# pzimbrod/fem-glass-tempering

Measured on AMD Instinct MI355X. Metric: DOF-updates/sec (coupled thermo-visco time step, 3D CG1 hex), higher is better.
Workload: dtype f64; 1 GPU; C4 3D plate CG1/CG1 400x400x50 hex (8200851 T-dofs), dt 0.1, coupled 6-term Prony; parallelism=single GPU, one partition (no communication), output=none (reference writes VTX/XDMF every step), krylov_form=PETSc KSPCG, geometric-multigrid V-cycle preconditioner, preconditioner=gmg, visco_fields=state (T, Tf, Tf_partial, phi, xi, s_tilde, sigma_tilde, sigma)

## Files before the change

### fem-glass-tempering_amd/csrc/tv_internal.h

```cpp
#pragma once
#include <hip/hip_runtime.h>
#include <cstdint>
#include <string>
#include <type_traits>
#include <vector>

#include "tvfem.h"

namespace tv {

constexpr int kWave = 64;
constexpr int kSeg = kWave - 2;
constexpr int kBlock = 256;

enum { kMemDoubles = 0, kMemOther = 1 };
template <class T>
constexpr int mem_kind() {
  return std::is_same<T, double>::value ? kMemDoubles : kMemOther;
}
hipError_t tv_dev_alloc(void** p, size_t bytes, int kind);
hipError_t tv_dev_free(void* p);
template <class T>
inline hipError_t tv_dev_alloc(T** p, size_t bytes, int kind) {
  void* q = nullptr;
// ... 263 lines not shown
                       const double* gface, double omega, double* r, double* dx, double* x0, int it_host, int init,
                       hipStream_t s);
int launch_dg_bpost(const DgGrid& g, const PcgState* st, const double* x0, const double* r, const double* w,
                    const double* gface, double omega, double* z, double* partials, const RedTail* tail, hipStream_t s);

void launch_visco(int dim, int all, const ViscoConst& c, const ViscoFields& f, hipStream_t s);
void launch_visco_Tpass(int dim, int all, const ViscoConst& c, const ViscoFields& f, hipStream_t s);
void launch_visco_Spass(int dim, int all, const ViscoConst& c, const ViscoFields& f, hipStream_t s);

struct EnsArgs {
  int n_bars, nb_pad, n_nodes;
  int n_steps;
  int step_base;
  int thermal_only;
  int max_it;
  double rtol, atol;
  double dt, sigma_sb;
  const double* cm;
  const double* ck;
  const double* htc;
  const double* T_amb;
  const double* eps;
  const double* f;
  double* T;
  double* Tp;
  double* scr;
  int* its_last;
  int* failed_step;
  int64_t* newton_total;
};
struct EnsExt {
  int n_stages;
  int n_probes;
  int every, max_records;
  const int* stage_end;
  const double* htc;
  const double* T_amb;
  const double* eps;
  const int* probes;
  double* hist;
};
void launch_ensemble(const EnsArgs& a, const ViscoConst& c, const ViscoFields& f, const EnsExt* x, hipStream_t s);
void launch_ensemble_dg(const EnsArgs& a, const ViscoConst& c, const ViscoFields& f, const EnsExt* x, hipStream_t s);

constexpr int kVecBlocks = 1024;
constexpr int kVecBlocksMin = 256;
constexpr int kVecNodesPerThread = 16;
constexpr int kVecBlocksMax = 8192;
void launch_pcg_init(int64_t n, const double* r, const double* dinv, double* z, double* dx,
                     double* partials, hipStream_t s);
struct FaceAdd {
  int on;
  int n0, n1, n2;
  int64_t t_off;
  double inv_n0, inv_plane;
  const double* ff[6];
};
FaceAdd cg_face_add(const CgGrid& g, int64_t t_off);


struct MgXfer {
  int fn[3], cn[3];
  int coarse[3];
  int f_kb, f_ke, c_kb, c_ke;
  const int* pi[3];
  const double* pw[3];
  const int* ri[3];
  const double* rw[3];
  int aligned;
};
void launch_mg_restrict(const MgXfer& x, const PcgState* st, const double* bf, const double* wf, const FaceAdd* fa,
                        const double* mask, double* bc, const double* dinv_c, double omega_c, double* xc,
                        hipStream_t s);
struct RRAxis {
  const int* f0;
  const double* w;
};
struct RRArgs {
  int on;
  int fn[3], cn[3];
  RRAxis ax[3];
  double da;
  int raxis, nseg, qchunk;
};
constexpr int kRRQMaxChunk = 64;
bool launch_mg_rrestrict(const RRArgs& a, const PcgState* st, const double* b, const double* x, const FaceAdd& fa,
                         double* bc, const double* dinv_c, double omega_c, double* xc, hipStream_t s);
void launch_cg_facet_faces(const CgGrid& g, const double* T, const double* x, const PcgState* st, hipStream_t s);
FaceAdd cg_face_add_all(const CgGrid& g);

struct CoarsePost {
  const double* b;
  const double* w;
  const double* dinv;
  double omega;
  FaceAdd fa;
};
void launch_mg_prolong(const MgXfer& x, const PcgState* st, double* xf, const double* xc, const double* mask,
                       hipStream_t s, const CoarsePost* cp = nullptr);
bool mg_prolong_smooths(const MgXfer& x);
bool mg_restrict_folds_faces(const MgXfer& x);
void launch_mg_jacobi(int64_t n, const PcgState* st, const double* b, const double* w, const FaceAdd* fa,
                      const double* dinv, double omega, double* x, int mode, hipStream_t s);
void launch_mg_inject(const MgXfer& x, const double* Tf, double* Tc, hipStream_t s);
void launch_mg_inject_range(const MgXfer& x, const double* Tf, double* Tc, int k0, int k1, hipStream_t s);
void launch_mg_resid(int64_t n, const PcgState* st, const double* b, double* w, const FaceAdd* fa, const double* mask,
                     hipStream_t s);
void launch_mg_ownmask(int64_t n, int64_t own0, int64_t own1, const double* dinv, double* mask, hipStream_t s);
constexpr int kMgPrepMax = 4;
struct MgPrep {
  int nlev;
  const double* Tbase;
  MgXfer xf[kMgPrepMax];
  double* T[kMgPrepMax];
  double* dinv[kMgPrepMax];
  CgGrid g[kMgPrepMax];
  int64_t off_n[kMgPrepMax + 1];
  int64_t off_b[kMgPrepMax + 1];
};
void launch_mg_prepare(const MgPrep& p, hipStream_t s);
bool cg_uses_march(const CgGrid& g);
void launch_mg_dg_restrict(const DgGrid& g, const PcgState* st, const double* bf, const double* wf, const double* mask,
                           double* bc, const double* dinv_c, double omega_c, double* xc, int kg0, hipStream_t s);
void launch_mg_dg_prolong(const DgGrid& g, const PcgState* st, double* xf, const double* xc, const double* mask,
                          int kg0, hipStream_t s);
void launch_mg_dg_T(const DgGrid& g, const double* Tdg, double* Tcg, int kg0, hipStream_t s);
int launch_mg_pow(int64_t n, const double* dinv, double* y, double* partials, hipStream_t s);
void launch_mg_scale(int64_t n, const double* y, double a, double* x, hipStream_t s);
bool launch_cg_japply_tail(const CgGrid& g, const double* T, const double* x, double* y, const PcgState* st,
                           double* partials, const RedTail* tail, hipStream_t s);
void launch_cg_japply_partial(const CgGrid& g, const double* T, const double* x, double* y, const PcgState* st,
                              hipStream_t s);
void launch_mg_update(int64_t n, const PcgState* st, const double* pA, const double* pB, const double* w,
                      const FaceAdd* fa, const double* dinv, double omega, double* r, double* dx, double* x0,
                      int it_host, int init, hipStream_t s, const double* lag = nullptr,
                      unsigned* counter = nullptr);
void launch_mg_update_cgs(int64_t n, const PcgState* st, const double* u, double* s, const double* z, double* p,
                          double* dx, double* r, const double* dinv, double omega, double* x0, bool first,
                          const double* lag, int lag_kind, unsigned* counter, hipStream_t stream);
int launch_cg_japply_post(const CgGrid& g, const double* T, const double* x, const double* r, const double* dinv,
                          double omega, double* z, const PcgState* st, double* partials, const RedTail* tail,
                          hipStream_t s);
int launch_mg_post(int64_t n, const PcgState* st, const double* x0, const double* r, const double* w,
                   const FaceAdd* fa, const double* dinv, double omega, double* z, double* partials,
                   const RedTail* tail, hipStream_t s);

void launch_pcg_update(int64_t n, PcgState* st, const double* pA, const double* pB, const double* w,
                       const double* dinv, double* dx, double* z, double* partials, hipStream_t s,
                       const RedTail* tail = nullptr, const FaceAdd* fa = nullptr, int it_host = 0);
void launch_pcg_dx_tail(int64_t n, const PcgState* st, const double* pA, const double* pB, double* dx, int its,
                        hipStream_t s);
void launch_mg_dx_finish(int64_t n, const PcgState* st, const double* pA, const double* pB, double* dx, int its,
                         hipStream_t s);
void launch_reduce_logic(const double* partials, int n, int W, double* out, PcgState* st, int kind,
                         int check_done, hipStream_t s);
void launch_logic(PcgState* st, const double* sums, int kind, hipStream_t s);
void launch_set_state(PcgState* st, const PcgState& h, hipStream_t s, const double* gate = nullptr);
void launch_newton_update(int64_t n, double* T, const double* dx, double* partials, hipStream_t s,
                          const RedTail* tail = nullptr);
void launch_post_group(int64_t n, const PcgState* st, const double* pA, const double* pB, double* dx, double* T,
                       double* partials, double* sums, hipStream_t s);
int pcg_vec_blocks(int64_t n);
void launch_fill(double* x, int64_t n, double v, hipStream_t s);

struct Output;
Output* output_create(const std::string& dir, int dim, const std::vector<std::vector<double>>& Xs, const int* phys,
                      std::string& err);
Output* output_create_unstructured(const std::string& dir, int dim, const std::vector<double>& xyz,
// ... 13 lines not shown
```

### fem-glass-tempering_amd/csrc/tv_mg.hip

```cpp
#include <algorithm>
#include <cstdlib>
#include <type_traits>

#include "tv_stencil.h"

namespace tv {
namespace {

template <bool MASK>
__global__ __launch_bounds__(kBlock) void k_mg_restrict(MgXfer x, const PcgState* __restrict__ st,
                                                        const double* __restrict__ bf,
                                                        const double* __restrict__ wf,
                                                        const double* __restrict__ mask, double* __restrict__ bc,
                                                        const double* __restrict__ dinv_c, double omega_c,
                                                        double* __restrict__ xc) {
  if (st != nullptr && st->done) return;
  const int plane = x.cn[0] * x.cn[1];
  const int n = plane * (x.c_ke - x.c_kb);
  const int fpl = x.fn[0] * x.fn[1];
  const int per = (n + (int)gridDim.x - 1) / (int)gridDim.x;
  const int t0 = xcd_remap(blockIdx.x, gridDim.x) * per, t1 = min(n, t0 + per);
  int k = (t0 + (int)threadIdx.x) / plane, j, i;
  {
    const int rem = t0 + (int)threadIdx.x - k * plane;
// ... 528 lines not shown
      if (xc != nullptr) xc[o] = omega_c * dinv_c[o] * acc;
    }
  };
  if (mask != nullptr) run(std::true_type{});
  else run(std::false_type{});
}

__global__ __launch_bounds__(kBlock) void k_mg_dg_prolong(DgGrid g, const PcgState* __restrict__ st,
                                                          double* __restrict__ xf, const double* __restrict__ xc,
                                                          const double* __restrict__ mask, int ck0, int ck1, int kg0) {
  if (st != nullptr && st->done) return;
  const int c0 = g.c0, c1 = g.c1, n0 = c0 + 1, n1 = c1 + 1;
  const int64_t pc = (int64_t)c0 * c1, ncell = pc * (ck1 - ck0);
  auto run = [&](auto masked) {
    constexpr bool MASKED = decltype(masked)::value;
    for (int64_t cell = blockIdx.x * (int64_t)kBlock + threadIdx.x; cell < ncell; cell += (int64_t)gridDim.x * kBlock) {
      const int i = (int)(cell % c0), j = (int)((cell / c0) % c1), k = ck0 + (int)(cell / pc);
      const DgL a = dg_lay(g, k);
      double xv[8], cv[8], mv[8];
#pragma unroll
      for (int l = 0; l < 8; ++l) {
        const int64_t v = (i + (l & 1)) + (int64_t)n0 * ((j + ((l >> 1) & 1)) + (int64_t)n1 * (k + kg0 + (l >> 2)));
        const int64_t f = a.base + (int64_t)l * a.stride + i + (int64_t)c0 * j;
        xv[l] = xf[f];
        cv[l] = xc[v];
        mv[l] = MASKED ? mask[f] : 1.0;
      }
#pragma unroll
      for (int l = 0; l < 8; ++l) {
        const int64_t f = a.base + (int64_t)l * a.stride + i + (int64_t)c0 * j;
        xf[f] = (MASKED && mv[l] == 0.0) ? 0.0 : xv[l] + cv[l];
      }
    }
  };
  if (mask != nullptr) run(std::true_type{});
  else run(std::false_type{});
}

__global__ __launch_bounds__(kBlock) void k_mg_dg_T(DgGrid g, const double* __restrict__ Tdg, double* __restrict__ Tcg,
                                                    int v0, int v1, int kg0) {
  const int c0 = g.c0, c1 = g.c1, c2 = g.c2, n0 = c0 + 1, n1 = c1 + 1;
  const int64_t nv = (int64_t)n0 * n1 * (v1 - v0);
  for (int64_t v = blockIdx.x * (int64_t)kBlock + threadIdx.x; v < nv; v += (int64_t)gridDim.x * kBlock) {
    const int i = (int)(v % n0), j = (int)((v / n0) % n1), K = v0 + (int)(v / ((int64_t)n0 * n1));
    double s = 0.0;
    int cnt = 0;
#pragma unroll
    for (int l = 0; l < 8; ++l) {
      const int ci = i - (l & 1), cj = j - ((l >> 1) & 1), ck = K - (l >> 2);
      if (ci < 0 || ci >= c0 || cj < 0 || cj >= c1 || ck < 0 || ck >= c2) continue;
      const DgL a = dg_lay(g, ck);
      s += Tdg[a.base + (int64_t)l * a.stride + ci + (int64_t)c0 * cj];
      ++cnt;
    }
    Tcg[i + (int64_t)n0 * (j + (int64_t)n1 * (K + kg0))] = s / cnt;
  }
}

__global__ __launch_bounds__(kBlock) void k_mg_pow(int64_t n, const double* __restrict__ dinv, double* __restrict__ y,
                                                   double* __restrict__ partials) {
  __shared__ double red[kBlock / kWave];
  double acc = 0.0;
  for (int64_t t = blockIdx.x * (int64_t)kBlock + threadIdx.x; t < n; t += (int64_t)gridDim.x * kBlock) {
    const double v = dinv ? dinv[t] * y[t] : y[t];
    y[t] = v;
    acc += v * v;
  }
  acc = wave_sum64(acc);
  if ((threadIdx.x & 63) == 0) red[threadIdx.x >> 6] = acc;
  __syncthreads();
  if (threadIdx.x == 0) partials[blockIdx.x] = (red[0] + red[1]) + (red[2] + red[3]);
}

__global__ __launch_bounds__(kBlock) void k_mg_scale(int64_t n, const double* __restrict__ y, double a,
                                                     double* __restrict__ x) {
  for (int64_t t = blockIdx.x * (int64_t)kBlock + threadIdx.x; t < n; t += (int64_t)gridDim.x * kBlock) x[t] = a * y[t];
}

int blocks_for(int64_t n) { return (int)std::max<int64_t>(1, std::min<int64_t>((n + kBlock - 1) / kBlock, 8192)); }
int xfer_blocks(int64_t n) { return (int)std::max<int64_t>(1, (n + kBlock - 1) / kBlock); }

constexpr int kRRSeg = kWave - 2;
constexpr int kRRWaves = 8;
constexpr int kRRRows = 2 * kRRWaves + 3;
constexpr int kRRPer = (kRRRows + kRRWaves - 1) / kRRWaves;
constexpr int kRRQMax = kRRQMaxChunk;
constexpr int kRRPF = 1;

using rr_buf = __amdgpu_buffer_rsrc_t;
__device__ __forceinline__ rr_buf rr_rsrc(const void* p, uint32_t bytes) {
  const uint64_t a = (uint64_t)p;
  const uint32_t lo = __builtin_amdgcn_readfirstlane((uint32_t)a);
  const uint32_t hi = __builtin_amdgcn_readfirstlane((uint32_t)(a >> 32));
  void* q = (void*)(((uint64_t)hi << 32) | lo);
  return __builtin_amdgcn_make_buffer_rsrc(q, (short)0, (int)__builtin_amdgcn_readfirstlane(bytes), 0x00020000);
}
__device__ __forceinline__ d2a8 rr_ld2(rr_buf r, uint32_t voff, uint32_t soff) {
  typedef unsigned int u4 __attribute__((ext_vector_type(4)));
  const u4 v = __builtin_amdgcn_raw_buffer_load_b128(r, (int)voff, (int)soff, 0);
  return __builtin_bit_cast(d2a8, v);
}
__device__ __forceinline__ d2a8 rr_tail(d2a8 v, bool tail) { return tail ? d2a8{v.y, 0.0} : v; }
__device__ __forceinline__ double rr_ld1(rr_buf r, uint32_t voff) {
  return __builtin_bit_cast(double, __builtin_amdgcn_raw_buffer_load_b64(r, (int)voff, 0, 0));
}

struct RRSet {
  d2a8 xv[kRRPer], bv[kRRPer];
  double fx[kRRPer];
  d2a8 fr;
};

template <int RA>
__global__ __launch_bounds__(kRRWaves * kWave) void k_mg_rrestrict(RRArgs a, const PcgState* __restrict__ st,
                                                                   const double* __restrict__ b,
                                                                   const double* __restrict__ x, FaceAdd fa,
                                                                   double* __restrict__ bc,
                                                                   const double* __restrict__ dinv_c, double omega_c,
                                                                   double* __restrict__ xc) {
  if (st != nullptr && st->done) return;
  __shared__ double sq[kRRQMax][15];
  __shared__ double sr[kRRWaves][15];
  __shared__ double red[2][3][kRRRows][kWave];
  const int lane = threadIdx.x & (kWave - 1);
  const int wave = __builtin_amdgcn_readfirstlane((int)threadIdx.x >> 6);
  constexpr int ra = RA, qa = 3 - RA;
  const int ncr = a.cn[ra], ncq = a.cn[qa];
  const int nrb = (ncr + kRRWaves - 1) / kRRWaves;
  const int bid = xcd_remap(blockIdx.x, gridDim.x);
  const int seg = bid % a.nseg;
  const int t = bid / a.nseg;
  const int rb = t % nrb, chunk = t / nrb;
  const int Jc0 = rb * kRRWaves;
  const int Jc = Jc0 + wave;
  const bool row_ok = Jc < ncr;
  const int Jcc = row_ok ? Jc : ncr - 1;
  const int Q0 = chunk * a.qchunk, Q1 = min(Q0 + a.qchunk, ncq);
  const int nf0 = a.fn[0], ncx = a.cn[0];
  const int nfr = a.fn[ra], nfq = a.fn[qa];
  const int I = seg * kRRSeg - 1 + lane;
  const bool Iok = I >= 0 && I < ncx;
  const int e0 = 2 * I;
  {
    const int tid = threadIdx.x;
    for (int e = tid; e < 15 * (Q1 - Q0); e += kRRWaves * kWave) sq[e / 15][e % 15] = a.ax[qa].w[15 * Q0 + e];
    if (lane < 15) sr[wave][lane] = row_ok ? a.ax[ra].w[15 * Jcc + lane] : 0.0;
  }
  const int Jlast = min(Jc0 + kRRWaves, ncr) - 1;
  const int fr_first = kld(a.ax[ra].f0, Jc0);
  const int nrows = kld(a.ax[ra].f0, Jlast) + 5 - fr_first;
  const int my0 = kld(a.ax[ra].f0, Jcc) - fr_first;
  const int sR = (ra == 1) ? nf0 : nf0 * a.fn[1];
  const int sQ = (ra == 1) ? nf0 * a.fn[1] : nf0;
  int frow[kRRPer];
  uint32_t rowoff[kRRPer];
  bool rload[kRRPer];
#pragma unroll
  for (int u = 0; u < kRRPer; ++u) {
    const int sl = wave + u * kRRWaves;
    rload[u] = sl < nrows;
    frow[u] = min(max(fr_first + sl, 0), nfr - 1);
    rowoff[u] = (uint32_t)(sR * frow[u]) * 8u;
  }
  const uint32_t nbytes = (uint32_t)a.fn[0] * (uint32_t)a.fn[1] * (uint32_t)a.fn[2] * 8u;
  const rr_buf rx = rr_rsrc(x, nbytes), rbv = rr_rsrc(b, nbytes);
  const bool xtail = Iok && e0 == nf0 - 1;
  const uint32_t voff = Iok ? (uint32_t)(e0 - (xtail ? 1 : 0)) * 8u : 0x40000000u;
  const bool xl0 = fa.ff[0] != nullptr && e0 == 0, xl1 = fa.ff[1] != nullptr && e0 == nf0 - 1;
  const int n1 = a.fn[1];
  const double* fxb = fa.ff[0] ? fa.ff[0] : fa.ff[1];
  const int64_t dx1 = (fa.ff[0] && fa.ff[1]) ? (int64_t)(fa.ff[1] - fa.ff[0]) : 0;
  const rr_buf rfx = rr_rsrc(fxb, fxb ? (uint32_t)((dx1 + (int64_t)n1 * a.fn[2]) * 8) : 0u);
  const uint32_t fxo = xl1 ? (uint32_t)dx1 : 0u;
  const uint32_t nfa = nbytes / (uint32_t)nfr, nfb = nbytes / (uint32_t)nfq;
  const rr_buf frl = rr_rsrc(fa.ff[2 * ra], fa.ff[2 * ra] ? nfa : 0u);
  const rr_buf frh = rr_rsrc(fa.ff[2 * ra + 1], fa.ff[2 * ra + 1] ? nfa : 0u);
  const rr_buf fql = rr_rsrc(fa.ff[2 * qa], fa.ff[2 * qa] ? nfb : 0u);
  const rr_buf fqh = rr_rsrc(fa.ff[2 * qa + 1], fa.ff[2 * qa + 1] ? nfb : 0u);
  const bool hrl = fa.ff[2 * ra] != nullptr, hrh = fa.ff[2 * ra + 1] != nullptr;
  const bool hql = fa.ff[2 * qa] != nullptr, hqh = fa.ff[2 * qa + 1] != nullptr;
  int uf = -1;
  bool uf_lo = false;
#pragma unroll
  for (int u = 0; u < kRRPer; ++u) {
    const int fr = fr_first + wave + u * kRRWaves;
    if (rload[u] && ((hrl && fr == 0) || (hrh && fr == nfr - 1))) {
      uf = u;
      uf_lo = hrl && fr == 0;
    }
  }
  const rr_buf frs = uf_lo ? frl : frh;
  const int f0q = kld(a.ax[qa].f0, Q0);
  const int np = 2 * (Q1 - Q0) + 3;
  auto fetch = [&](int P, RRSet& S) {
    const int fq = min(max(f0q + P, 0), nfq - 1);
    const uint32_t po = (uint32_t)(sQ * fq) * 8u;
#pragma unroll
    for (int u = 0; u < kRRPer; ++u) {
      S.xv[u] = rr_ld2(rx, rload[u] ? voff : 0x40000000u, rowoff[u] + po);
      S.bv[u] = rr_ld2(rbv, rload[u] ? voff : 0x40000000u, rowoff[u] + po);
    }
#pragma unroll
    for (int u = 0; u < kRRPer; ++u) {
      const int j = (ra == 1) ? frow[u] : fq, k = (ra == 1) ? fq : frow[u];
      S.fx[u] = rr_ld1(rfx, ((xl0 || xl1) && rload[u]) ? (fxo + (uint32_t)(j + n1 * k)) * 8u : 0x40000000u);
    }
    S.fr = rr_ld2(frs, uf >= 0 ? voff : 0x40000000u, (uint32_t)(nf0 * fq) * 8u);
  };
  double wx[15];
#pragma unroll
  for (int m = 0; m < 15; ++m) wx[m] = (Iok ? a.ax[0].w[15 * (Iok ? I : 0) + m] : 0.0);
  auto reduce = [&](int P, const RRSet& S) {
    const int fqr = f0q + P;
    const bool qlo = hql && fqr == 0, qhi = hqh && fqr == nfq - 1;
    d2a8 sv[kRRPer];
#pragma unroll
    for (int u = 0; u < kRRPer; ++u) {
      sv[u] = rr_tail(S.bv[u], xtail);
      sv[u].x -= S.fx[u];
      if (u == uf) {
        const d2a8 f = rr_tail(S.fr, xtail);
        sv[u].x -= f.x;
        sv[u].y -= f.y;
      }
      if (qlo || qhi) {
        const d2a8 f = rr_tail(rr_ld2(qlo ? fql : fqh, voff, (uint32_t)(nf0 * frow[u]) * 8u), xtail);
        sv[u].x -= f.x;
        sv[u].y -= f.y;
      }
    }
    const int buf = P & 1;
#pragma unroll
    for (int u = 0; u < kRRPer; ++u) {
      const d2a8 xv = rr_tail(S.xv[u], xtail);
      const double x0 = shr1(xv.x), x1 = shr1(xv.y), x4 = shl1(xv.x);
      const double s0 = shr1(sv[u].x), s1 = shr1(sv[u].y), s4 = shl1(sv[u].x);
      const double p = ((wx[0] * x0 + wx[1] * x1) + wx[2] * xv.x) + (wx[3] * xv.y + wx[4] * x4);
      const double q = ((wx[5] * x0 + wx[6] * x1) + wx[7] * xv.x) + (wx[8] * xv.y + wx[9] * x4);
      const double s = ((wx[10] * s0 + wx[11] * s1) + wx[12] * sv[u].x) + (wx[13] * sv[u].y + wx[14] * s4);
      const int sl = wave + u * kRRWaves;
      if (sl < kRRRows) {
        red[buf][0][sl][lane] = p;
        red[buf][1][sl][lane] = q;
        red[buf][2][sl][lane] = s;
      }
    }
  };
  auto fold = [&](int P, double& U, double& V, double& Sv) {
    const int buf = P & 1;
    double um = 0.0, uk = 0.0, vv = 0.0, ss = 0.0;
#pragma unroll
    for (int m = 0; m < 5; ++m) {
      const int sl = min(my0 + m, kRRRows - 1);
      const double p = red[buf][0][sl][lane], q = red[buf][1][sl][lane], s = red[buf][2][sl][lane];
      um += sr[wave][m] * (p + a.da * q);
      uk += sr[wave][5 + m] * p;
      vv += sr[wave][m] * p;
      ss += sr[wave][10 + m] * s;
    }
    U = um + a.da * uk;
    V = vv;
    Sv = ss;
  };
  auto contrib = [&](int Q, int m, double U, double V, double Sv) {
    const double* w = sq[Q - Q0];
    return w[10 + m] * Sv - (w[m] * U + a.da * (w[5 + m] * V));
  };
  const bool out_lane = row_ok && Iok && lane >= 1 && lane <= kRRSeg;
  const int nQ = Q1 - Q0;
  double X = 0.0, Y = 0.0;
  const uint32_t ncb = (uint32_t)ncx * (uint32_t)a.cn[1] * (uint32_t)a.cn[2] * 8u;
  const rr_buf rdc = rr_rsrc(dinv_c, xc != nullptr ? ncb : 0u);
  auto coarse_off = [&](int Q) -> uint32_t {
    const int J1 = (ra == 1) ? Jc : Q, K2 = (ra == 1) ? Q : Jc;
    return ((uint32_t)I + (uint32_t)ncx * ((uint32_t)J1 + (uint32_t)a.cn[1] * (uint32_t)K2)) * 8u;
  };
  RRSet S[kRRPF + 1];
#pragma unroll
  for (int s = 0; s < kRRPF; ++s) fetch(min(s, np - 1), S[s]);
  __syncthreads();
#pragma unroll 1
  for (int P0 = 0; P0 < np; P0 += kRRPF + 1) {
#pragma unroll
    for (int s = 0; s <= kRRPF; ++s) {
      const int P = P0 + s;
      const bool completes = P < np && (P & 1) == 0 && (P >> 1) - 2 >= 0 && out_lane;
      const double dcv = rr_ld1(rdc, completes ? coarse_off(Q0 + (P >> 1) - 2) : 0x40000000u);
      __builtin_amdgcn_sched_barrier(0);
      fetch(min(P + kRRPF, np - 1), S[(s + kRRPF) % (kRRPF + 1)]);
      if (P < np) {
        reduce(P, S[s]);
        __syncthreads();
        double U, V, Sv;
        fold(P, U, V, Sv);
        const int k = P >> 1;
        if ((P & 1) == 0) {
          if (k - 2 >= 0 && k - 2 < nQ) X += contrib(Q0 + k - 2, 4, U, V, Sv);
          if (k - 1 >= 0 && k - 1 < nQ) Y += contrib(Q0 + k - 1, 2, U, V, Sv);
          const double Z = (k < nQ) ? contrib(Q0 + k, 0, U, V, Sv) : 0.0;
          if (completes) {
            const int64_t o = coarse_off(Q0 + k - 2) / 8u;
            bc[o] = X;
            if (xc != nullptr) xc[o] = omega_c * dcv * X;
          }
          X = Y;
          Y = Z;
        } else {
          if (k - 1 >= 0 && k - 1 < nQ) X += contrib(Q0 + k - 1, 3, U, V, Sv);
          if (k < nQ) Y += contrib(Q0 + k, 1, U, V, Sv);
        }
      }
    }
  }
}

}



void launch_mg_restrict(const MgXfer& x, const PcgState* st, const double* bf, const double* wf, const FaceAdd* fa,
                        const double* mask, double* bc, const double* dinv_c, double omega_c, double* xc,
                        hipStream_t s) {
  const bool faces = fa != nullptr && fa->on;
  const int64_t n = (int64_t)x.cn[0] * x.cn[1] * (x.c_ke - x.c_kb);
  if (n <= 0) return;
  if (mg_restrict_folds_faces(x)) {
    const int nseg = (x.cn[0] + kPairSeg - 1) / kPairSeg;
    const dim3 g((unsigned)((int64_t)x.cn[1] * (x.c_ke - x.c_kb) * nseg));
    const FaceAdd f = faces ? *fa : FaceAdd{};
#define TV_RP(M, F) \
  hipLaunchKernelGGL((k_mg_restrict_pairs<M, F>), g, dim3(kWave), 0, s, x, st, bf, wf, mask, bc, dinv_c, omega_c, xc, \
                     nseg, f)
    if (mask != nullptr) {
      if (faces) TV_RP(true, true);
      else TV_RP(true, false);
    } else {
      if (faces) TV_RP(false, true);
      else TV_RP(false, false);
    }
#undef TV_RP
    return;
  }
  if (mask != nullptr)
    hipLaunchKernelGGL(k_mg_restrict<true>, dim3(xfer_blocks(n)), dim3(kBlock), 0, s, x, st, bf, wf, mask, bc, dinv_c,
                       omega_c, xc);
  else
    hipLaunchKernelGGL(k_mg_restrict<false>, dim3(xfer_blocks(n)), dim3(kBlock), 0, s, x, st, bf, wf, mask, bc,
                       dinv_c, omega_c, xc);
}

bool mg_restrict_folds_faces(const MgXfer& x) { return x.coarse[0] && x.fn[0] >= 3; }

bool launch_mg_rrestrict(const RRArgs& a, const PcgState* st, const double* b, const double* x, const FaceAdd& fa,
                         double* bc, const double* dinv_c, double omega_c, double* xc, hipStream_t s) {
  const int ncr = a.cn[a.raxis], ncq = a.cn[3 - a.raxis];
  const int nrb = (ncr + kRRWaves - 1) / kRRWaves;
  if (a.qchunk < 1 || a.qchunk > kRRQMax) return false;
  const int nch = (ncq + a.qchunk - 1) / a.qchunk;
  const dim3 g((unsigned)((int64_t)a.nseg * nrb * nch)), bl(kRRWaves * kWave);
  if (a.raxis == 1) hipLaunchKernelGGL(k_mg_rrestrict<1>, g, bl, 0, s, a, st, b, x, fa, bc, dinv_c, omega_c, xc);
  else hipLaunchKernelGGL(k_mg_rrestrict<2>, g, bl, 0, s, a, st, b, x, fa, bc, dinv_c, omega_c, xc);
  return true;
}

bool mg_prolong_blocks(const MgXfer& x) {
  return x.aligned && x.coarse[0] && x.coarse[1] && x.coarse[2] && x.fn[0] >= 3 && x.f_kb == 0;
}

bool mg_prolong_smooths(const MgXfer& x) { return mg_prolong_blocks(x); }

void launch_mg_prolong(const MgXfer& x, const PcgState* st, double* xf, const double* xc, const double* mask,
                       hipStream_t s, const CoarsePost* cp) {
  const int64_t n = (int64_t)x.fn[0] * x.fn[1] * (x.f_ke - x.f_kb);
  if (n <= 0) return;
  if (cp != nullptr && !mg_prolong_smooths(x)) {
    const int64_t nc = (int64_t)x.cn[0] * x.cn[1] * x.cn[2];
    launch_mg_jacobi(nc, st, cp->b, cp->w, &cp->fa, cp->dinv, cp->omega, const_cast<double*>(xc), 1, s);
    cp = nullptr;
  }
  if (mg_prolong_blocks(x)) {
    const int nseg = ((x.fn[0] + 1) / 2 + kPairSeg - 1) / kPairSeg;
    const int nbj = (x.fn[1] + 1) / 2, nbk = (x.f_ke + 1) / 2;
    if (cp != nullptr)
      hipLaunchKernelGGL(k_mg_prolong_blk<true>, dim3((unsigned)((int64_t)nbj * nbk * nseg)), dim3(kWave), 0, s, x, st,
                         xf, xc, mask, nseg, nbj, *cp);
    else
      hipLaunchKernelGGL(k_mg_prolong_blk<false>, dim3((unsigned)((int64_t)nbj * nbk * nseg)), dim3(kWave), 0, s, x, st,
                         xf, xc, mask, nseg, nbj, CoarsePost{});
    return;
  }
  if (x.coarse[0] && x.fn[0] >= 3) {
    const int nseg = ((x.fn[0] + 1) / 2 + kPairSeg - 1) / kPairSeg;
    const int64_t rows = (int64_t)x.fn[1] * (x.f_ke - x.f_kb);
    hipLaunchKernelGGL(k_mg_prolong_pairs, dim3((unsigned)(rows * nseg)), dim3(kWave), 0, s, x, st, xf, xc, mask, nseg);
    return;
  }
  hipLaunchKernelGGL(k_mg_prolong, dim3((unsigned)((n + kPU * kBlock - 1) / (kPU * kBlock))), dim3(kBlock), 0, s, x, st, xf, xc, mask);
}

void launch_mg_jacobi(int64_t n, const PcgState* st, const double* b, const double* w, const FaceAdd* fa,
                      const double* dinv, double omega, double* x, int mode, hipStream_t s) {
  if (n <= 0) return;
  const FaceAdd f = (fa && fa->on) ? *fa : FaceAdd{};
  const dim3 g(blocks_for(n)), bl(kBlock);
  if (mode == 0) hipLaunchKernelGGL((k_mg_jacobi<0, false>), g, bl, 0, s, n, st, b, w, f, dinv, omega, x);
  else if (f.on) hipLaunchKernelGGL((k_mg_jacobi<1, true>), g, bl, 0, s, n, st, b, w, f, dinv, omega, x);
  else hipLaunchKernelGGL((k_mg_jacobi<1, false>), g, bl, 0, s, n, st, b, w, f, dinv, omega, x);
}

void launch_mg_inject(const MgXfer& x, const double* Tf, double* Tc, hipStream_t s) {
  launch_mg_inject_range(x, Tf, Tc, 0, x.cn[2], s);
}

void launch_mg_inject_range(const MgXfer& x, const double* Tf, double* Tc, int k0, int k1, hipStream_t s) {
  const int nxb = (x.cn[0] + kBlock - 1) / kBlock;
  const int64_t rows = (int64_t)x.cn[1] * (k1 - k0);
  if (rows > 0) hipLaunchKernelGGL(k_mg_inject, dim3((unsigned)(rows * nxb)), dim3(kBlock), 0, s, x, Tf, Tc, nxb, k0);
}

void launch_mg_resid(int64_t n, const PcgState* st, const double* b, double* w, const FaceAdd* fa, const double* mask,
                     hipStream_t s) {
  if (n <= 0) return;
  const FaceAdd f = (fa && fa->on) ? *fa : FaceAdd{};
  if (f.on) hipLaunchKernelGGL((k_mg_resid<true>), dim3(blocks_for(n)), dim3(kBlock), 0, s, n, st, b, w, f, mask);
  else hipLaunchKernelGGL((k_mg_resid<false>), dim3(blocks_for(n)), dim3(kBlock), 0, s, n, st, b, w, f, mask);
}

void launch_mg_ownmask(int64_t n, int64_t own0, int64_t own1, const double* dinv, double* mask, hipStream_t s) {
  if (n <= 0) return;
  hipLaunchKernelGGL(k_mg_ownmask, dim3(blocks_for(n)), dim3(kBlock), 0, s, n, own0, own1, dinv, mask);
}

void launch_mg_dg_restrict(const DgGrid& g, const PcgState* st, const double* bf, const double* wf, const double* mask,
                           double* bc, const double* dinv_c, double omega_c, double* xc, int kg0, hipStream_t s) {
  const int64_t nv = (int64_t)(g.c0 + 1) * (g.c1 + 1) * (g.k_end - g.k_begin + 1);
  hipLaunchKernelGGL(k_mg_dg_restrict, dim3(blocks_for(nv)), dim3(kBlock), 0, s, g, st, bf, wf, mask, bc, dinv_c,
                     omega_c, xc, g.k_begin, g.k_end + 1, g.k_begin, g.k_end, kg0);
}

void launch_mg_dg_prolong(const DgGrid& g, const PcgState* st, double* xf, const double* xc, const double* mask,
                          int kg0, hipStream_t s) {
  const int64_t nc = (int64_t)g.c0 * g.c1 * g.c2;
// ... 21 lines not shown
```

### fem-glass-tempering_amd/csrc/tv_mgsolve.cpp

```cpp
#include <cstdlib>

#include "tv_ctx.h"

namespace tv {
constexpr int64_t kMgFoldFacesNodes = 4000000;

double mg_gershgorin(const std::vector<double> (&X)[3], double dt_alpha) {
  using Row = std::array<double, 6>;
  std::vector<Row> rows[3];
  for (int s = 0; s < 3; ++s) {
    std::vector<double> cf;
    axis_coefs(X[s], 0, (int)X[s].size(), cf);
    for (size_t i = 0; i < X[s].size(); ++i) {
      const double* c = &cf[i * C_NCOEF];
      rows[s].push_back({c[C_MLO], c[C_MDI], c[C_MUP], c[C_KLO], c[C_KDI], c[C_KUP]});
    }
    std::sort(rows[s].begin(), rows[s].end());
    rows[s].erase(std::unique(rows[s].begin(), rows[s].end()), rows[s].end());
  }
  double b = 0.0;
  for (const Row& r0 : rows[0])
    for (const Row& r1 : rows[1])
      for (const Row& r2 : rows[2]) {
        double sum = 0.0, diag = 0.0;
// ... 126 lines not shown
      pw[2 * i] = 1.0;
    } else {
      const double wl = (Xf[i + 1] - Xf[i]) / (Xf[i + 1] - Xf[i - 1]);
      pi[2 * i] = cpos[i - 1];
      pi[2 * i + 1] = cpos[i + 1];
      pw[2 * i] = wl;
      pw[2 * i + 1] = 1.0 - wl;
    }
  }
  for (int I = 0; I < nc; ++I) {
    const int fc = fpos[I];
    for (int q = 0; q < 3; ++q) ri[3 * I + q] = fc;
    rw[3 * I + 1] = 1.0;
    if (fc - 1 >= 0 && !is_c[fc - 1]) {
      ri[3 * I] = fc - 1;
      rw[3 * I] = pw[2 * (fc - 1) + 1];
    }
    if (fc + 1 < nf && !is_c[fc + 1]) {
      ri[3 * I + 2] = fc + 1;
      rw[3 * I + 2] = pw[2 * (fc + 1)];
    }
  }
}

static bool rr_axis(const std::vector<double>& Xf, const std::vector<int>& ri, const std::vector<double>& rw,
                    std::vector<int>& f0, std::vector<double>& w) {
  const int nf = (int)Xf.size(), nc = (int)ri.size() / 3;
  std::vector<double> cf;
  axis_coefs(Xf, 0, nf, cf);
  f0.assign(nc, 0);
  w.assign(15 * (size_t)nc, 0.0);
  for (int I = 0; I < nc; ++I) {
    f0[I] = ri[3 * I + 1] - 2;
    for (int q = 0; q < 3; ++q) {
      const int f = ri[3 * I + q];
      const double wt = rw[3 * I + q];
      if (wt == 0.0) continue;
      const double* cc = &cf[(size_t)f * C_NCOEF];
      auto add = [&](int col, int fi, double v) -> bool {
        if (v == 0.0) return true;
        const int m = fi - f0[I];
        if (fi < 0 || fi >= nf || m < 0 || m > 4) return false;
        w[15 * (size_t)I + 5 * col + m] += wt * v;
        return true;
      };
      if (!(add(0, f - 1, cc[C_MLO]) && add(0, f, cc[C_MDI]) && add(0, f + 1, cc[C_MUP]) &&
            add(1, f - 1, cc[C_KLO]) && add(1, f, cc[C_KDI]) && add(1, f + 1, cc[C_KUP]) && add(2, f, 1.0)))
        return false;
    }
  }
  return true;
}

static int rr_setup(Ctx* c, MgLevel& L, const std::vector<double> (&Xp)[3], const std::vector<int> (&ri)[3],
                    const std::vector<double> (&rw)[3]) {
  RRArgs& a = L.rr;
  a = RRArgs{};
  const MgXfer& x = L.xf;
  if (!x.coarse[0] || x.fn[0] < 5 || !(x.fn[0] & 1)) return TV_OK;
  std::vector<int> f0[3];
  std::vector<double> w[3];
  for (int s = 0; s < 3; ++s)
    if (!rr_axis(Xp[s], ri[s], rw[s], f0[s], w[s])) return TV_OK;
  auto regular = [&](int s) {
    if (!x.coarse[s] || x.cn[s] < 2) return false;
    for (int I = 0; I + 1 < x.cn[s]; ++I)
      if (f0[s][I + 1] - f0[s][I] != 2) return false;
    return true;
  };
  int qa = (x.cn[1] <= x.cn[2]) ? 1 : 2;
  if (!regular(qa)) qa = 3 - qa;
  if (!regular(qa)) return TV_OK;
  a.raxis = 3 - qa;
  for (int I = 0; I + 1 < x.cn[a.raxis]; ++I)
    if (f0[a.raxis][I + 1] - f0[a.raxis][I] > 2) return TV_OK;
  for (int s = 0; s < 3; ++s) {
    a.fn[s] = x.fn[s];
    a.cn[s] = x.cn[s];
    if (int e = mg_upload(c, L, f0[s], &a.ax[s].f0)) return e;
    if (int e = mg_upload(c, L, w[s], &a.ax[s].w)) return e;
  }
  a.da = L.g.dt_alpha;
  a.nseg = (x.cn[0] + 61) / 62;
  const char* te = std::getenv("TVFEM_RR_WG");
  const int target = te ? std::max(1, std::atoi(te)) : 256;
  const int64_t rowblocks = (x.cn[a.raxis] + 7) / 8;
  a.qchunk = std::min(x.cn[qa], kRRQMaxChunk);
  while ((int64_t)a.nseg * rowblocks * ((x.cn[qa] + a.qchunk - 1) / a.qchunk) < target && a.qchunk > 3)
    a.qchunk = (a.qchunk + 1) / 2;
  if (a.qchunk < 1 || a.qchunk > kRRQMaxChunk)
    return c->fail(TV_ERR_STATE, "GMG: fused residual restriction: march chunk " + std::to_string(a.qchunk) +
                                     " outside [1, " + std::to_string(kRRQMaxChunk) + "]");
  a.on = 1;
  return TV_OK;
}

constexpr int64_t kRRMinNodes = 3000000;
static unsigned rr_levels(int64_t fine_nodes) {
  const char* e = std::getenv("TVFEM_MG_RR");
  if (e) return (unsigned)std::strtoul(e, nullptr, 0);
  return fine_nodes >= kRRMinNodes ? 1u : 0u;
}

int mg_level_vectors(Ctx* c, MgLevel& L) {
  const CgGrid& f = c->cg;
  L.g.dt = f.dt; L.g.dt_alpha = f.dt_alpha; L.g.dt_f = f.dt_f;
  L.g.a_rad = f.a_rad; L.g.a_conv = f.a_conv; L.g.T_amb = f.T_amb; L.g.T_amb4 = f.T_amb4;
  L.n = (int64_t)L.g.n0 * L.g.n1 * L.g.n2;
  for (double** q : {&L.T, &L.b, &L.x, &L.w, &L.dinv}) {
    void* p = nullptr;
    HIPC(tv_dev_alloc(&p, sizeof(double) * (size_t)std::max<int64_t>(1, L.n), kMemDoubles));
    HIPC(hipMemsetAsync(p, 0, sizeof(double) * (size_t)std::max<int64_t>(1, L.n), c->stream));
    L.bufs.push_back(p);
    *q = static_cast<double*>(p);
  }
  return TV_OK;
}

int mg_setup(Ctx* c) {
  const bool dg = c->fam_T == TV_DG;
  if (c->dim != 3 || c->um || (!dg && !cg_cgs_supported(c->cg)) || (dg && (c->dg.deg1 || c->dg.deg2)))
    return c->fail(TV_ERR_ARG, "preconditioner GMG: 3D CG1 or DG1 temperature space on a rectilinear mesh only");
  if (c->cgs) return c->fail(TV_ERR_ARG, "preconditioner GMG runs in the KSPCG form (pcg_variant KSPCG or AUTO)");
  if (c->n_parts > 1 && !dg) return mg_setup_dist(c);
  if (c->n_parts > 1) c->mg_A = 1;
  std::vector<double> tmp, Xf[3];
  for (int s = 0; s < 3; ++s) Xf[s] = storage_coords(c, s, tmp);
  const double da = c->P.dt * c->P.alpha;
  HIPC(tv_dev_alloc(&c->mgx, sizeof(double) * (size_t)std::max<int64_t>(1, c->nT), kMemDoubles));
  HIPC(hipMemsetAsync(c->mgx, 0, sizeof(double) * (size_t)std::max<int64_t>(1, c->nT), c->stream));
  if (dg) {
    c->mg_dg = true;
    HIPC(tv_dev_alloc(&c->dggface, sizeof(double) * (size_t)dg_gface_size(c->dg), kMemDoubles));
    c->mg_omega0 = 0.0;
    if (int e = mg_add_cg_level(c, Xf, da)) return e;
  } else {
    c->mg_omega0 = mg_omega(mg_gershgorin(Xf, da));
  }
  const int max_levels = c->O.mg_levels > 0 ? c->O.mg_levels : 8;
  const bool automatic = c->O.mg_levels <= 0;
  std::vector<double> Xp[3] = {Xf[0], Xf[1], Xf[2]};
  for (int lev = 1 + (dg ? 1 : 0); lev < max_levels; ++lev) {
    std::vector<double> Xc[3];
    std::vector<char> is_c[3];
    int coarse[3];
    if (!mg_next_level(Xp, da, automatic, Xc, is_c, coarse)) break;
    c->mg.emplace_back();
    MgLevel& L = c->mg.back();
    for (int s = 0; s < 3; ++s) L.X[s] = Xc[s];
    if (int e = build_cg_grid(c, 3, L.X, 0, (int)L.X[2].size(), 0, 0, true, true, L.g, L.coef, &L.bnodes, L.ffbuf))
      return e;
    if (int e = mg_level_vectors(c, L)) return e;
    L.omega = mg_omega(mg_gershgorin(L.X, da));
    MgXfer& x = L.xf;
    std::vector<int> ri[3];
    std::vector<double> rw[3];
    for (int s = 0; s < 3; ++s) {
      std::vector<int> pi;
      std::vector<double> pw;
      mg_axis_tables(Xp[s], is_c[s], pi, pw, ri[s], rw[s]);
      if (int e = mg_upload(c, L, pi, &x.pi[s])) return e;
      if (int e = mg_upload(c, L, pw, &x.pw[s])) return e;
      if (int e = mg_upload(c, L, ri[s], &x.ri[s])) return e;
      if (int e = mg_upload(c, L, rw[s], &x.rw[s])) return e;
      x.fn[s] = (int)Xp[s].size();
      x.cn[s] = (int)L.X[s].size();
      x.coarse[s] = coarse[s];
    }
    x.f_kb = 0;
    x.f_ke = x.fn[2];
    x.c_kb = 0;
    x.c_ke = x.cn[2];
// ... 295 lines not shown
```

Baseline: 849.5 million DOF-updates/s.

## Retile fused residual restriction to fold six coarse rows per workgroup, sized to CU count

The fused residual-restriction kernel now folds six coarse rows per workgroup instead of eight. This shrinks the shared fine-row buffer and the reduction slots, and leaves the extra waves to do loading and reduction only. The march-chunk sizing targets two workgroups per CU using the device CU count and balances chunk lengths, where it used to aim for a fixed 256 workgroups. It also adds launch bounds for occupancy, handles a second boundary face row per wave, and adds a scheduling barrier after prefetch. The aim is better occupancy and load balance across CUs, at the cost of more halo rows re-read per coarse row.

```diff
diff --git a/fem-glass-tempering_amd/csrc/tv_internal.h b/fem-glass-tempering_amd/csrc/tv_internal.h
--- a/fem-glass-tempering_amd/csrc/tv_internal.h
+++ b/fem-glass-tempering_amd/csrc/tv_internal.h
@@ -369,8 +369,11 @@
   RRAxis ax[3];
   double da;
   int raxis, nseg, qchunk;
+  int nrb, nch;
 };
 constexpr int kRRQMaxChunk = 64;
+constexpr int kRRFold = 6;
+constexpr int kRRWgPerCU = 2;
 bool launch_mg_rrestrict(const RRArgs& a, const PcgState* st, const double* b, const double* x, const FaceAdd& fa,
                          double* bc, const double* dinv_c, double omega_c, double* xc, hipStream_t s);
 void launch_cg_facet_faces(const CgGrid& g, const double* T, const double* x, const PcgState* st, hipStream_t s);
diff --git a/fem-glass-tempering_amd/csrc/tv_mg.hip b/fem-glass-tempering_amd/csrc/tv_mg.hip
--- a/fem-glass-tempering_amd/csrc/tv_mg.hip
+++ b/fem-glass-tempering_amd/csrc/tv_mg.hip
@@ -634,10 +634,11 @@
 
 constexpr int kRRSeg = kWave - 2;
 constexpr int kRRWaves = 8;
-constexpr int kRRRows = 2 * kRRWaves + 3;
+constexpr int kRRRows = 2 * kRRFold + 3;
 constexpr int kRRPer = (kRRRows + kRRWaves - 1) / kRRWaves;
 constexpr int kRRQMax = kRRQMaxChunk;
 constexpr int kRRPF = 1;
+static_assert(kRRFold <= kRRWaves, "a wave folds at most one coarse row");
 
 using rr_buf = __amdgpu_buffer_rsrc_t;
 __device__ __forceinline__ rr_buf rr_rsrc(const void* p, uint32_t bytes) {
@@ -664,7 +665,7 @@
 };
 
 template <int RA>
-__global__ __launch_bounds__(kRRWaves * kWave) void k_mg_rrestrict(RRArgs a, const PcgState* __restrict__ st,
+__global__ __launch_bounds__(kRRWaves * kWave, 2 * kRRWgPerCU) void k_mg_rrestrict(RRArgs a, const PcgState* __restrict__ st,
                                                                    const double* __restrict__ b,
                                                                    const double* __restrict__ x, FaceAdd fa,
                                                                    double* __restrict__ bc,
@@ -672,20 +673,20 @@
                                                                    double* __restrict__ xc) {
   if (st != nullptr && st->done) return;
   __shared__ double sq[kRRQMax][15];
-  __shared__ double sr[kRRWaves][15];
+  __shared__ double sr[kRRFold][15];
   __shared__ double red[2][3][kRRRows][kWave];
   const int lane = threadIdx.x & (kWave - 1);
   const int wave = __builtin_amdgcn_readfirstlane((int)threadIdx.x >> 6);
   constexpr int ra = RA, qa = 3 - RA;
   const int ncr = a.cn[ra], ncq = a.cn[qa];
-  const int nrb = (ncr + kRRWaves - 1) / kRRWaves;
+  const int nrb = a.nrb;
   const int bid = xcd_remap(blockIdx.x, gridDim.x);
   const int seg = bid % a.nseg;
   const int t = bid / a.nseg;
   const int rb = t % nrb, chunk = t / nrb;
-  const int Jc0 = rb * kRRWaves;
+  const int Jc0 = rb * kRRFold;
   const int Jc = Jc0 + wave;
-  const bool row_ok = Jc < ncr;
+  const bool row_ok = wave < kRRFold && Jc < ncr;
   const int Jcc = row_ok ? Jc : ncr - 1;
   const int Q0 = chunk * a.qchunk, Q1 = min(Q0 + a.qchunk, ncq);
   const int nf0 = a.fn[0], ncx = a.cn[0];
@@ -696,9 +697,9 @@
   {
     const int tid = threadIdx.x;
     for (int e = tid; e < 15 * (Q1 - Q0); e += kRRWaves * kWave) sq[e / 15][e % 15] = a.ax[qa].w[15 * Q0 + e];
-    if (lane < 15) sr[wave][lane] = row_ok ? a.ax[ra].w[15 * Jcc + lane] : 0.0;
-  }
-  const int Jlast = min(Jc0 + kRRWaves, ncr) - 1;
+    if (row_ok && lane < 15) sr[wave][lane] = a.ax[ra].w[15 * Jc + lane];
+  }
+  const int Jlast = min(Jc0 + kRRFold, ncr) - 1;
   const int fr_first = kld(a.ax[ra].f0, Jc0);
   const int nrows = kld(a.ax[ra].f0, Jlast) + 5 - fr_first;
   const int my0 = kld(a.ax[ra].f0, Jcc) - fr_first;
@@ -731,14 +732,18 @@
   const rr_buf fqh = rr_rsrc(fa.ff[2 * qa + 1], fa.ff[2 * qa + 1] ? nfb : 0u);
   const bool hrl = fa.ff[2 * ra] != nullptr, hrh = fa.ff[2 * ra + 1] != nullptr;
   const bool hql = fa.ff[2 * qa] != nullptr, hqh = fa.ff[2 * qa + 1] != nullptr;
-  int uf = -1;
+  int uf = -1, uf2 = -1;
   bool uf_lo = false;
 #pragma unroll
   for (int u = 0; u < kRRPer; ++u) {
     const int fr = fr_first + wave + u * kRRWaves;
     if (rload[u] && ((hrl && fr == 0) || (hrh && fr == nfr - 1))) {
-      uf = u;
-      uf_lo = hrl && fr == 0;
+      if (uf < 0) {
+        uf = u;
+        uf_lo = hrl && fr == 0;
+      } else {
+        uf2 = u;
+      }
     }
   }
   const rr_buf frs = uf_lo ? frl : frh;
@@ -775,6 +780,12 @@
         sv[u].x -= f.x;
         sv[u].y -= f.y;
       }
+      if (u == uf2) {
+        const int fq = min(max(fqr, 0), nfq - 1);
+        const d2a8 f = rr_tail(rr_ld2(frh, voff, (uint32_t)(nf0 * fq) * 8u), xtail);
+        sv[u].x -= f.x;
+        sv[u].y -= f.y;
+      }
       if (qlo || qhi) {
         const d2a8 f = rr_tail(rr_ld2(qlo ? fql : fqh, voff, (uint32_t)(nf0 * frow[u]) * 8u), xtail);
         sv[u].x -= f.x;
@@ -784,18 +795,17 @@
     const int buf = P & 1;
 #pragma unroll
     for (int u = 0; u < kRRPer; ++u) {
+      const int sl = wave + u * kRRWaves;
+      if ((u + 1) * kRRWaves > kRRRows && sl >= kRRRows) continue;
       const d2a8 xv = rr_tail(S.xv[u], xtail);
       const double x0 = shr1(xv.x), x1 = shr1(xv.y), x4 = shl1(xv.x);
       const double s0 = shr1(sv[u].x), s1 = shr1(sv[u].y), s4 = shl1(sv[u].x);
       const double p = ((wx[0] * x0 + wx[1] * x1) + wx[2] * xv.x) + (wx[3] * xv.y + wx[4] * x4);
       const double q = ((wx[5] * x0 + wx[6] * x1) + wx[7] * xv.x) + (wx[8] * xv.y + wx[9] * x4);
       const double s = ((wx[10] * s0 + wx[11] * s1) + wx[12] * sv[u].x) + (wx[13] * sv[u].y + wx[14] * s4);
-      const int sl = wave + u * kRRWaves;
-      if (sl < kRRRows) {
-        red[buf][0][sl][lane] = p;
-        red[buf][1][sl][lane] = q;
-        red[buf][2][sl][lane] = s;
-      }
+      red[buf][0][sl][lane] = p;
+      red[buf][1][sl][lane] = q;
+      red[buf][2][sl][lane] = s;
     }
   };
   auto fold = [&](int P, double& U, double& V, double& Sv) {
@@ -829,7 +839,10 @@
   };
   RRSet S[kRRPF + 1];
 #pragma unroll
-  for (int s = 0; s < kRRPF; ++s) fetch(min(s, np - 1), S[s]);
+  for (int s = 0; s < kRRPF; ++s) {
+    fetch(min(s, np - 1), S[s]);
+    __builtin_amdgcn_sched_barrier(0);
+  }
   __syncthreads();
 #pragma unroll 1
   for (int P0 = 0; P0 < np; P0 += kRRPF + 1) {
@@ -843,6 +856,7 @@
       if (P < np) {
         reduce(P, S[s]);
         __syncthreads();
+        if (!row_ok) continue;
         double U, V, Sv;
         fold(P, U, V, Sv);
         const int k = P >> 1;
@@ -905,11 +919,8 @@
 
 bool launch_mg_rrestrict(const RRArgs& a, const PcgState* st, const double* b, const double* x, const FaceAdd& fa,
                          double* bc, const double* dinv_c, double omega_c, double* xc, hipStream_t s) {
-  const int ncr = a.cn[a.raxis], ncq = a.cn[3 - a.raxis];
-  const int nrb = (ncr + kRRWaves - 1) / kRRWaves;
   if (a.qchunk < 1 || a.qchunk > kRRQMax) return false;
-  const int nch = (ncq + a.qchunk - 1) / a.qchunk;
-  const dim3 g((unsigned)((int64_t)a.nseg * nrb * nch)), bl(kRRWaves * kWave);
+  const dim3 g((unsigned)((int64_t)a.nseg * a.nrb * a.nch)), bl(kRRWaves * kWave);
   if (a.raxis == 1) hipLaunchKernelGGL(k_mg_rrestrict<1>, g, bl, 0, s, a, st, b, x, fa, bc, dinv_c, omega_c, xc);
   else hipLaunchKernelGGL(k_mg_rrestrict<2>, g, bl, 0, s, a, st, b, x, fa, bc, dinv_c, omega_c, xc);
   return true;
diff --git a/fem-glass-tempering_amd/csrc/tv_mgsolve.cpp b/fem-glass-tempering_amd/csrc/tv_mgsolve.cpp
--- a/fem-glass-tempering_amd/csrc/tv_mgsolve.cpp
+++ b/fem-glass-tempering_amd/csrc/tv_mgsolve.cpp
@@ -232,12 +232,16 @@
   }
   a.da = L.g.dt_alpha;
   a.nseg = (x.cn[0] + 61) / 62;
+  int cus = 0;
+  HIPC(hipDeviceGetAttribute(&cus, hipDeviceAttributeMultiprocessorCount, c->device));
   const char* te = std::getenv("TVFEM_RR_WG");
-  const int target = te ? std::max(1, std::atoi(te)) : 256;
-  const int64_t rowblocks = (x.cn[a.raxis] + 7) / 8;
-  a.qchunk = std::min(x.cn[qa], kRRQMaxChunk);
-  while ((int64_t)a.nseg * rowblocks * ((x.cn[qa] + a.qchunk - 1) / a.qchunk) < target && a.qchunk > 3)
-    a.qchunk = (a.qchunk + 1) / 2;
+  const int64_t target = te ? std::max(1, std::atoi(te)) : (int64_t)kRRWgPerCU * std::max(1, cus);
+  const int ncq = x.cn[qa];
+  a.nrb = (x.cn[a.raxis] + kRRFold - 1) / kRRFold;
+  const int64_t fit = std::max<int64_t>(1, std::min<int64_t>(target / ((int64_t)a.nseg * a.nrb), ncq));
+  a.qchunk = std::min(std::max((int)((ncq + fit - 1) / fit), std::min(3, ncq)), kRRQMaxChunk);
+  a.nch = (ncq + a.qchunk - 1) / a.qchunk;
+  a.qchunk = (ncq + a.nch - 1) / a.nch;
   if (a.qchunk < 1 || a.qchunk > kRRQMaxChunk)
     return c->fail(TV_ERR_STATE, "GMG: fused residual restriction: march chunk " + std::to_string(a.qchunk) +
                                      " outside [1, " + std::to_string(kRRQMaxChunk) + "]");
```

After: 861.2 million DOF-updates/s (median of 6 runs). 1.4% higher.
